# zhaoruiyang98/eftpipe

Measured on AMD Instinct MI355X. Metric: theory P_l(k) evaluations/sec (single tracer, Nk=512, l=0,2,4), higher is better.
Workload: dtype f64

## Files before the change

### eftpipe_amd/csrc/eftb_kernels.hpp

```cpp
#pragma once
#include <hip/hip_runtime.h>
#include <stdint.h>
#include <stdlib.h>

namespace eftb {

constexpr int NS = 80;
constexpr int NPOW = 257;
constexpr int NHALF = 128;
constexpr int NCH = 129;

constexpr int NROW = 24;

typedef double v4d __attribute__((ext_vector_type(4)));
typedef double v2d __attribute__((ext_vector_type(2)));

__device__ __forceinline__ void xcd_decode(int ntile, int& tile, int& group) {
    const int flat = blockIdx.x, ng = gridDim.x / ntile;
    if ((ng & 7) == 0) {
        const int slot = flat >> 3;
        tile = slot % ntile;
        group = (flat & 7) + 8 * (slot / ntile);
    } else {
        tile = flat % ntile;
        group = flat / ntile;
    }
}

template <bool LO>
__device__ __forceinline__ void prep_rows_body(int Nkin, int ntail, int nxtail, int KP1, int KP2, int KP3, int Bmax,
                                                        const double* __restrict__ Pin, const double* __restrict__ lnkin,
                                                        const double* __restrict__ lnxtail, const double* __restrict__ lnxxtail,
                                                        const double* __restrict__ wq2, double* __restrict__ A1, double* __restrict__ A2,
                                                        double* __restrict__ A2T, double* __restrict__ A3, int* __restrict__ status,
                                                        int ntail_lo, int nxtail_lo) {
    extern __shared__ double sm[];
    double* pin = sm;
    const int w = blockIdx.x, tid = threadIdx.x;
    bool bad = false;
    for (int j = tid; j < Nkin; j += blockDim.x) {
        const double v = Pin[(size_t)w * Nkin + j];
        pin[j] = v;
        bad = bad || !(fabs(v) <= 1.79769313486231570815e308) || (j >= Nkin - 2 && !(v > 0.0));
        if (LO) bad = bad || (j < 2 && !(v > 0.0));
    }
    if (bad && status) atomicMax(status, w + 1);
    __syncthreads();
    const double dln = lnkin[Nkin - 1] - lnkin[Nkin - 2];
    const double dlo = LO ? lnkin[1] - lnkin[0] : 0.0;
    if (A1) {
        const double slope = (log(pin[Nkin - 1]) - log(pin[Nkin - 2])) / dln;
        const double amp = pin[Nkin - 1] * exp(-slope * lnkin[Nkin - 1]);
        double slo = 0.0, alo = 0.0;
        if (LO && ntail_lo) {
            slo = (log(pin[1]) - log(pin[0])) / dlo;
            alo = pin[0] * exp(-slo * lnkin[0]);
        }
        const int nhi = ntail - (LO ? ntail_lo : 0);
        for (int j = tid; j < KP1; j += blockDim.x) A1[(size_t)w * KP1 + j] = j < Nkin ? pin[j] : 0.0;
        for (int j = tid; j < KP2; j += blockDim.x) {
            double v = j < Nkin ? pin[j] : (j < Nkin + ntail ? amp * exp(slope * lnxtail[j - Nkin]) : 0.0);
            if (LO && j >= Nkin + nhi && j < Nkin + ntail) v = alo * exp(slo * lnxtail[j - Nkin]);
            A2[(size_t)w * KP2 + j] = v;
            A2T[(size_t)j * Bmax + w] = v;
        }
    }
    if (A3) {
        const double q1 = pin[Nkin - 1] * wq2[1], q0 = pin[Nkin - 2] * wq2[0];
        const double slope = (log(q1) - log(q0)) / dln;
        const double amp = q1 * exp(-slope * lnkin[Nkin - 1]);
        double slo = 0.0, alo = 0.0;
        if (LO && nxtail_lo) {
            const double p0 = pin[0] * wq2[2], p1 = pin[1] * wq2[3];
            slo = (log(p1) - log(p0)) / dlo;
            alo = p0 * exp(-slo * lnkin[0]);
        }
        const int nhi = nxtail - (LO ? nxtail_lo : 0);
        for (int j = tid; j < KP3; j += blockDim.x) {
            double v = j < Nkin ? pin[j] : (j < Nkin + nxtail ? amp * exp(slope * lnxxtail[j - Nkin]) : 0.0);
            if (LO && j >= Nkin + nhi && j < Nkin + nxtail) v = alo * exp(slo * lnxxtail[j - Nkin]);
            A3[(size_t)w * KP3 + j] = v;
        }
    }
}

#define PREP_ROWS_PARAMS int Nkin, int ntail, int nxtail, int KP1, int KP2, int KP3, int Bmax, const double* __restrict__ Pin, \
    const double* __restrict__ lnkin, const double* __restrict__ lnxtail, const double* __restrict__ lnxxtail, const double* __restrict__ wq2, \
    double* __restrict__ A1, double* __restrict__ A2, double* __restrict__ A2T, double* __restrict__ A3, int* __restrict__ status
#define PREP_ROWS_ARGS Nkin, ntail, nxtail, KP1, KP2, KP3, Bmax, Pin, lnkin, lnxtail, lnxxtail, wq2, A1, A2, A2T, A3, status

__global__ __launch_bounds__(256) void prep_rows_kernel(PREP_ROWS_PARAMS) {
    prep_rows_body<false>(PREP_ROWS_ARGS, 0, 0);
}

__global__ __launch_bounds__(256) void prep_rows_lo_kernel(PREP_ROWS_PARAMS, int ntail_lo, int nxtail_lo) {
    prep_rows_body<true>(PREP_ROWS_ARGS, ntail_lo, nxtail_lo);
}

__device__ __forceinline__ void qf_body(int w, int nq, const double* __restrict__ fgrow, const double* __restrict__ Qpoly, double* __restrict__ Q) {
    const int tid = threadIdx.x;
    const double f = fgrow[w];
    for (int idx = tid; idx < 2 * nq; idx += blockDim.x) {
        const int a = idx / nq, rest = idx % nq;
        const double* c = Qpoly + ((size_t)(1 - a) * nq + rest) * 15;
        double cv[15];
#pragma unroll
        for (int p = 0; p < 15; ++p) cv[p] = c[p];
        const double f2 = f * f;
        double ev = cv[14], od = cv[13];
#pragma unroll
        for (int p = 12; p >= 0; p -= 2) {
            ev = fma(ev, f2, cv[p]);
            if (p >= 1) od = fma(od, f2, cv[p - 1]);
        }
        Q[(size_t)w * 2 * nq + idx] = fma(od, f, ev);
    }
}

__global__ __launch_bounds__(256) void prep_rows_qf_kernel(int B, PREP_ROWS_PARAMS, int nq, const double* __restrict__ fgrow,
                                                           const double* __restrict__ Qpoly, double* __restrict__ Q) {
    if ((int)blockIdx.x >= B) {
        qf_body(blockIdx.x - B, nq, fgrow, Qpoly, Q);
        return;
    }
    prep_rows_body<false>(PREP_ROWS_ARGS, 0, 0);
}

__global__ __launch_bounds__(256) void prep_rows_qf_lo_kernel(int B, PREP_ROWS_PARAMS, int nq, const double* __restrict__ fgrow,
                                                              const double* __restrict__ Qpoly, double* __restrict__ Q, int ntail_lo, int nxtail_lo) {
    if ((int)blockIdx.x >= B) {
        qf_body(blockIdx.x - B, nq, fgrow, Qpoly, Q);
        return;
    }
    prep_rows_body<true>(PREP_ROWS_ARGS, ntail_lo, nxtail_lo);
}
#undef PREP_ROWS_PARAMS
#undef PREP_ROWS_ARGS

constexpr int AD_T = NHALF + 2;
constexpr int AD_CH = 1;
constexpr int KSYN = 528;
constexpr int KLIN = 288;
constexpr int SYN_KPAD = 48;
constexpr int SYN_KC = 24;
static_assert(SYN_KPAD % SYN_KC == 0 && (32 * SYN_KC) % 256 == 0, "chunk must divide the padding and fill the staging threads");
constexpr int BAS22 = 8, BASC = 32;

__device__ __forceinline__ double readlane_f64(double v, int lane) {
    return __hiloint2double(__builtin_amdgcn_readlane(__double2hiint(v), lane), __builtin_amdgcn_readlane(__double2loint(v), lane));
}

template <int NC, int NW>
__global__ __launch_bounds__(64 * NW) void antidiag_kernel(int B, int Bmax, const double* __restrict__ coefT,
                                                           const double2* __restrict__ AD, double2* __restrict__ S) {
    constexpr int PB = 3, WPP = 2 * NC;
    static_assert(PB * WPP <= 64, "one wave-load must hold a block's weights");
    __shared__ double red[NW - 1][2 * NC][64];
    const int grp = blockIdx.y, jp = (grp & 1) ? NPOW - 1 - (int)blockIdx.x : (int)blockIdx.x;
    const int lane = threadIdx.x & 63, wave = threadIdx.x >> 6, w = grp * 64 + lane;
    const int wl = w < B ? w : B - 1;
    const int cnt = ((2 * NHALF + jp) >> 1) - jp + 1;
    const int per = (cnt + NW - 1) / NW, t0 = wave * per, t1 = min(cnt, t0 + per);
    const double* cr = coefT + wl;
    const double* ci = coefT + (size_t)NCH * Bmax + wl;
    double ar[NC], ai[NC];
#pragma unroll
    for (int q = 0; q < NC; ++q) ar[q] = ai[q] = 0.0;
    if (t0 < t1) {
        const double* adw = reinterpret_cast<const double*>(AD + ((size_t)jp * AD_T + t0) * NC);
        const int nw = (t1 - t0) * WPP;
        auto wload = [&](int blk) { return adw[min(blk * PB * WPP + lane, nw - 1)]; };
        double xr[PB], xi[PB], yr[PB], yi[PB];
        auto coef = [&](int t, int p) {
            const int n = jp + t, qn = n <= NHALF ? n : 2 * NHALF - n;
            xr[p] = cr[(size_t)qn * Bmax];
            xi[p] = ci[(size_t)qn * Bmax];
            yr[p] = cr[(size_t)t * Bmax];
            yi[p] = ci[(size_t)t * Bmax];
        };
        double wc = wload(0);
#pragma unroll
        for (int p = 0; p < PB; ++p) coef(min(t0 + p, t1 - 1), p);
        const int nblk = (t1 - t0 + PB - 1) / PB;
        for (int blk = 0; blk < nblk; ++blk) {
            const double wn = wload(blk + 1);
#pragma unroll
            for (int p = 0; p < PB; ++p) {
                const int t = t0 + blk * PB + p;
                const double on = t < t1 ? 1.0 : 0.0;
                const double xim = jp + t <= NHALF ? xi[p] : -xi[p], yim = -yi[p];
                const double pr = (xr[p] * yr[p] - xim * yim) * on, pi = (xr[p] * yim + xim * yr[p]) * on;
                __builtin_amdgcn_sched_barrier(0);
                coef(min(t + PB, t1 - 1), p);
                __builtin_amdgcn_sched_barrier(0);
#pragma unroll
                for (int q = 0; q < NC; ++q) {
                    const double mx = readlane_f64(wc, p * WPP + 2 * q), my = readlane_f64(wc, p * WPP + 2 * q + 1);
                    ar[q] = fma(mx, pr, fma(-my, pi, ar[q]));
                    ai[q] = fma(mx, pi, fma(my, pr, ai[q]));
                }
                __builtin_amdgcn_sched_barrier(0);
            }
            wc = wn;
        }
    }
    if (wave > 0) {
#pragma unroll
        for (int q = 0; q < NC; ++q) {
            red[wave - 1][2 * q][lane] = ar[q];
            red[wave - 1][2 * q + 1][lane] = ai[q];
        }
    }
    __syncthreads();
    if (wave == 0 && w < B) {
#pragma unroll
        for (int q = 0; q < NC; ++q) {
#pragma unroll
            for (int v = 0; v < NW - 1; ++v) {
                ar[q] += red[v][2 * q][lane];
                ai[q] += red[v][2 * q + 1][lane];
            }
            S[((size_t)w * NC + q) * NPOW + jp] = make_double2(ar[q], ai[q]);
        }
    }
}

template <int NC, int NW>
__global__ __launch_bounds__(64 * NW) void antidiag_nh_kernel(int B, int Bmax, const double* __restrict__ coefT,
                                                              const double2* __restrict__ AD, double2* __restrict__ S, int nh) {
    constexpr int PB = 3, WPP = 2 * NC;
    static_assert(PB * WPP <= 64, "one wave-load must hold a block's weights");
    __shared__ double red[NW - 1][2 * NC][64];
    const int npow = 2 * nh + 1, nch = nh + 1, adt = nh + 2;
    const int grp = blockIdx.y, jp = (grp & 1) ? npow - 1 - (int)blockIdx.x : (int)blockIdx.x;
    const int lane = threadIdx.x & 63, wave = threadIdx.x >> 6, w = grp * 64 + lane;
    const int wl = w < B ? w : B - 1;
    const int cnt = ((2 * nh + jp) >> 1) - jp + 1;
    const int per = (cnt + NW - 1) / NW, t0 = wave * per, t1 = min(cnt, t0 + per);
    const double* cr = coefT + wl;
    const double* ci = coefT + (size_t)nch * Bmax + wl;
    double ar[NC], ai[NC];
#pragma unroll
    for (int q = 0; q < NC; ++q) ar[q] = ai[q] = 0.0;
    if (t0 < t1) {
        const double* adw = reinterpret_cast<const double*>(AD + ((size_t)jp * adt + t0) * NC);
        const int nw = (t1 - t0) * WPP;
        auto wload = [&](int blk) { return adw[min(blk * PB * WPP + lane, nw - 1)]; };
        double xr[PB], xi[PB], yr[PB], yi[PB];
        auto coef = [&](int t, int p) {
            const int n = jp + t, qn = n <= nh ? n : 2 * nh - n;
            xr[p] = cr[(size_t)qn * Bmax];
            xi[p] = ci[(size_t)qn * Bmax];
            yr[p] = cr[(size_t)t * Bmax];
            yi[p] = ci[(size_t)t * Bmax];
        };
        double wc = wload(0);
#pragma unroll
        for (int p = 0; p < PB; ++p) coef(min(t0 + p, t1 - 1), p);
        const int nblk = (t1 - t0 + PB - 1) / PB;
        for (int blk = 0; blk < nblk; ++blk) {
            const double wn = wload(blk + 1);
#pragma unroll
            for (int p = 0; p < PB; ++p) {
                const int t = t0 + blk * PB + p;
                const double on = t < t1 ? 1.0 : 0.0;
                const double xim = jp + t <= nh ? xi[p] : -xi[p], yim = -yi[p];
                const double pr = (xr[p] * yr[p] - xim * yim) * on, pi = (xr[p] * yim + xim * yr[p]) * on;
                __builtin_amdgcn_sched_barrier(0);
                coef(min(t + PB, t1 - 1), p);
                __builtin_amdgcn_sched_barrier(0);
#pragma unroll
                for (int q = 0; q < NC; ++q) {
                    const double mx = readlane_f64(wc, p * WPP + 2 * q), my = readlane_f64(wc, p * WPP + 2 * q + 1);
                    ar[q] = fma(mx, pr, fma(-my, pi, ar[q]));
                    ai[q] = fma(mx, pi, fma(my, pr, ai[q]));
                }
                __builtin_amdgcn_sched_barrier(0);
            }
            wc = wn;
        }
    }
    if (wave > 0) {
#pragma unroll
        for (int q = 0; q < NC; ++q) {
            red[wave - 1][2 * q][lane] = ar[q];
            red[wave - 1][2 * q + 1][lane] = ai[q];
        }
    }
    __syncthreads();
    if (wave == 0 && w < B) {
#pragma unroll
        for (int q = 0; q < NC; ++q) {
#pragma unroll
            for (int v = 0; v < NW - 1; ++v) {
                ar[q] += red[v][2 * q][lane];
                ai[q] += red[v][2 * q + 1][lane];
            }
            S[((size_t)w * NC + q) * npow + jp] = make_double2(ar[q], ai[q]);
        }
    }
}

template <int NC>
__global__ __launch_bounds__(64) void build_rows_kernel(int sets, int Bmax, int Nl, int nlc, int nb, const double* __restrict__ coef,
                                                         const double2* __restrict__ S, const double2* __restrict__ mlj,
                                                         const double2* __restrict__ linvec, double* __restrict__ A22,
                                                         double* __restrict__ A13, double* __restrict__ ACF, double* __restrict__ ALC) {
    const int w = blockIdx.x, cf = blockIdx.y, jp = blockIdx.z * 64 + threadIdx.x;
    if (((sets >> cf) & 1) && jp < NPOW) {
        double zr[NC], zi[NC];
#pragma unroll
        for (int q = 0; q < NC; ++q) {
            zr[q] = zi[q] = 0.0;
#pragma unroll
            for (int ch = 0; ch < AD_CH; ++ch) {
                const double2 v = S[(((size_t)ch * Bmax + w) * NC + q) * NPOW + jp];
                zr[q] += v.x;
                zi[q] += v.y;
            }
        }
        const int o0 = jp == 0 ? 0 : 2 * jp - 1;
        if (cf == 0) {
#pragma unroll
            for (int q = 0; q < NC; ++q)
                if (q < nb) {
                    double* o = A22 + ((size_t)w * BAS22 + q) * KSYN;
                    o[o0] = zr[q];
                    if (jp) o[o0 + 1] = zi[q];
                }
        } else {
            for (int l = 0; l < Nl; ++l) {
                const double2 m = mlj[l * NPOW + jp];
#pragma unroll
                for (int q = 0; q < NC; ++q) {
                    double* o = ACF + ((size_t)w * BASC + l * NC + q) * KSYN;
                    o[o0] = m.x * zr[q] - m.y * zi[q];
                    if (jp) o[o0 + 1] = m.x * zi[q] + m.y * zr[q];
                }
            }
        }
    }
    if ((sets >> (2 + cf)) & 1) {
        const int nrows = cf == 0 ? 10 : nlc * Nl, v0 = cf == 0 ? 0 : 10;
        double* out = cf == 0 ? A13 + (size_t)w * 10 * KLIN : ALC + (size_t)w * nlc * Nl * KLIN;
        const double* c = coef + (size_t)w * 2 * NCH;
        for (int e = jp; e < nrows * NCH; e += 320) {
            const int row = e / NCH, mp = e % NCH, n = NHALF - mp;
            const double2 v = linvec[(size_t)(v0 + row) * NCH + n];
            const double cr = c[n], ci = n == NHALF ? 0.0 : c[NCH + n];
            double* o = out + (size_t)row * KLIN;
            if (mp == 0) o[0] = cr * v.x - ci * v.y;
            else {
                o[2 * mp - 1] = cr * v.x - ci * v.y;
                o[2 * mp] = cr * v.y + ci * v.x;
            }
        }
    }
}

__host__ __device__ constexpr int ksyn_of(int nh) { return (4 * nh + SYN_KPAD) / SYN_KPAD * SYN_KPAD; }
__host__ __device__ constexpr int klin_of(int nh) { return (2 * nh + SYN_KPAD) / SYN_KPAD * SYN_KPAD; }
static_assert(ksyn_of(NHALF) == KSYN && klin_of(NHALF) == KLIN, "row lengths of the default NFFT");

template <int NC>
__global__ __launch_bounds__(64) void build_rows_nh_kernel(int sets, int Bmax, int Nl, int nlc, int nb, const double* __restrict__ coef,
                                                            const double2* __restrict__ S, const double2* __restrict__ mlj,
                                                            const double2* __restrict__ linvec, double* __restrict__ A22,
                                                            double* __restrict__ A13, double* __restrict__ ACF, double* __restrict__ ALC, int nh) {
    const int npow = 2 * nh + 1, nch = nh + 1, ksyn = ksyn_of(nh), klin = klin_of(nh), zstride = 64 * (int)gridDim.z;
    const int w = blockIdx.x, cf = blockIdx.y, jp = blockIdx.z * 64 + threadIdx.x;
    if (((sets >> cf) & 1) && jp < npow) {
        double zr[NC], zi[NC];
#pragma unroll
        for (int q = 0; q < NC; ++q) {
            zr[q] = zi[q] = 0.0;
#pragma unroll
            for (int ch = 0; ch < AD_CH; ++ch) {
                const double2 v = S[(((size_t)ch * Bmax + w) * NC + q) * npow + jp];
                zr[q] += v.x;
                zi[q] += v.y;
            }
        }
        const int o0 = jp == 0 ? 0 : 2 * jp - 1;
        if (cf == 0) {
#pragma unroll
            for (int q = 0; q < NC; ++q)
                if (q < nb) {
                    double* o = A22 + ((size_t)w * BAS22 + q) * ksyn;
                    o[o0] = zr[q];
                    if (jp) o[o0 + 1] = zi[q];
                }
        } else {
            for (int l = 0; l < Nl; ++l) {
                const double2 m = mlj[l * npow + jp];
#pragma unroll
                for (int q = 0; q < NC; ++q) {
                    double* o = ACF + ((size_t)w * BASC + l * NC + q) * ksyn;
                    o[o0] = m.x * zr[q] - m.y * zi[q];
                    if (jp) o[o0 + 1] = m.x * zi[q] + m.y * zr[q];
                }
            }
        }
    }
    if ((sets >> (2 + cf)) & 1) {
        const int nrows = cf == 0 ? 10 : nlc * Nl, v0 = cf == 0 ? 0 : 10;
        double* out = cf == 0 ? A13 + (size_t)w * 10 * klin : ALC + (size_t)w * nlc * Nl * klin;
        const double* c = coef + (size_t)w * 2 * nch;
        for (int e = jp; e < nrows * nch; e += zstride) {
            const int row = e / nch, mp = e % nch, n = nh - mp;
            const double2 v = linvec[(size_t)(v0 + row) * nch + n];
            const double cr = c[n], ci = n == nh ? 0.0 : c[nch + n];
            double* o = out + (size_t)row * klin;
            if (mp == 0) o[0] = cr * v.x - ci * v.y;
            else {
                o[2 * mp - 1] = cr * v.x - ci * v.y;
                o[2 * mp] = cr * v.y + ci * v.x;
            }
        }
    }
}

__device__ inline double ipow(double f, int p) {
    double r = 1.0;
    for (int i = 0; i < p; ++i) r *= f;
    return r;
}

template <int NC>
__global__ __launch_bounds__(64) void build_rows_plk_kernel(int Bmax, int nb, const double* __restrict__ coef, const double2* __restrict__ S,
                                                             const double2* __restrict__ mlj, const double2* __restrict__ linvec,
                                                             const double* __restrict__ bias, const double* __restrict__ fgrow,
                                                             const double* __restrict__ l11, const double* __restrict__ lct,
                                                             const double* __restrict__ l22, const double* __restrict__ l13,
                                                             const int* __restrict__ grp, const double* __restrict__ exp22,
                                                             const double* __restrict__ expc, double* __restrict__ A22, double* __restrict__ A13,
                                                             double* __restrict__ ACF, double* __restrict__ ALC) {
    constexpr int NL = 3;
    __shared__ double s_cf[NL * 38];
    __shared__ double s_w[NL * NC];
    __shared__ double s_b[2 * NL];
    const int w = blockIdx.x, cf = blockIdx.y, jp = blockIdx.z * 64 + threadIdx.x;
    const double* bw = bias + (size_t)w * NROW;
    const double f = fgrow[w];
    for (int e = threadIdx.x; e < NL * 38; e += 64) {
        const int l = e / 38, bq = e % 38;
        s_cf[e] = bw[9 + grp[2 * bq]] * ipow(f, grp[2 * bq + 1]) * (bq < 28 ? l22[l * 28 + bq] : l13[l * 10 + (bq - 28)]);
    }
    if (threadIdx.x < 2 * NL) {
        const int a = threadIdx.x / NL, lp = threadIdx.x % NL;
        double v = 0.0;
        if (a == 0)
            for (int r = 0; r < 3; ++r) v = fma(bw[r], l11[lp * 3 + r], v);
        else
            for (int r = 0; r < 6; ++r) v = fma(bw[3 + r], lct[lp * 6 + r], v);
        s_b[threadIdx.x] = v;
    }
    __syncthreads();
    if (threadIdx.x < NL * NC) {
        const int l = threadIdx.x / NC, q = threadIdx.x % NC;
        double v0 = 0.0, v1 = 0.0;
        if (cf == 0) {
            if (q < nb)
                for (int b = 0; b < 28; b += 2) {
                    v0 = fma(s_cf[l * 38 + b], exp22[b * BAS22 + q], v0);
                    v1 = fma(s_cf[l * 38 + b + 1], exp22[(b + 1) * BAS22 + q], v1);
                }
        } else {
            for (int b = 0; b < 28; b += 2) {
                v0 = fma(s_cf[l * 38 + b], expc[(size_t)(l * 28 + b) * BASC + l * NC + q], v0);
                v1 = fma(s_cf[l * 38 + b + 1], expc[(size_t)(l * 28 + b + 1) * BASC + l * NC + q], v1);
            }
            for (int b = 0; b < 10; b += 2) {
                v0 = fma(s_cf[l * 38 + 28 + b], expc[(size_t)(NL * 28 + l * 10 + b) * BASC + l * NC + q], v0);
                v1 = fma(s_cf[l * 38 + 29 + b], expc[(size_t)(NL * 28 + l * 10 + b + 1) * BASC + l * NC + q], v1);
            }
        }
        s_w[threadIdx.x] = v0 + v1;
    }
    __syncthreads();
    if (jp < NPOW) {
        double zr[NC], zi[NC];
#pragma unroll
        for (int q = 0; q < NC; ++q) {
            zr[q] = zi[q] = 0.0;
#pragma unroll
            for (int ch = 0; ch < AD_CH; ++ch) {
                const double2 v = S[(((size_t)ch * Bmax + w) * NC + q) * NPOW + jp];
                zr[q] += v.x;
                zi[q] += v.y;
            }
        }
        const int o0 = jp == 0 ? 0 : 2 * jp - 1;
#pragma unroll
        for (int l = 0; l < NL; ++l) {
            double cr = 0.0, ci = 0.0;
#pragma unroll
            for (int q = 0; q < NC; ++q) {
                cr = fma(s_w[l * NC + q], zr[q], cr);
                ci = fma(s_w[l * NC + q], zi[q], ci);
            }
            if (cf == 0) {
                double* o = A22 + ((size_t)w * BAS22 + l) * KSYN;
                o[o0] = cr;
                if (jp) o[o0 + 1] = ci;
            } else {
                const double2 m = mlj[l * NPOW + jp];
                double* o = ACF + ((size_t)w * BASC + l) * KSYN;
                o[o0] = m.x * cr - m.y * ci;
                if (jp) o[o0 + 1] = m.x * ci + m.y * cr;
            }
        }
    }
    {
        const int nrows = cf == 0 ? NL : 2 * NL;
        double* out = cf == 0 ? A13 + (size_t)w * 10 * KLIN : ALC + (size_t)w * 2 * NL * KLIN;
        const double* c = coef + (size_t)w * 2 * NCH;
        for (int e = jp; e < nrows * NCH; e += 320) {
            const int row = e / NCH, mp = e % NCH, n = NHALF - mp;
            double vx, vy;
            if (cf == 0) {
                vx = vy = 0.0;
#pragma unroll
                for (int b = 0; b < 10; ++b) {
                    const double2 v = linvec[(size_t)b * NCH + n];
                    vx = fma(s_cf[row * 38 + 28 + b], v.x, vx);
                    vy = fma(s_cf[row * 38 + 28 + b], v.y, vy);
                }
            } else {
                const double2 v = linvec[(size_t)(10 + row) * NCH + n];
                vx = s_b[row] * v.x;
                vy = s_b[row] * v.y;
            }
            const double cr = c[n], ci = n == NHALF ? 0.0 : c[NCH + n];
            double* o = out + (size_t)row * KLIN;
            if (mp == 0) o[0] = cr * vx - ci * vy;
            else {
                o[2 * mp - 1] = cr * vx - ci * vy;
                o[2 * mp] = cr * vy + ci * vx;
            }
        }
    }
}

template <int NC>
__global__ __launch_bounds__(64) void build_rows_plk_nh_kernel(int Bmax, int nb, const double* __restrict__ coef, const double2* __restrict__ S,
                                                    const double2* __restrict__ mlj, const double2* __restrict__ linvec,
                                                    const double* __restrict__ bias, const double* __restrict__ fgrow,
                                                    const double* __restrict__ l11, const double* __restrict__ lct,
                                                    const double* __restrict__ l22, const double* __restrict__ l13,
                                                    const int* __restrict__ grp, const double* __restrict__ exp22,
                                                    const double* __restrict__ expc, double* __restrict__ A22, double* __restrict__ A13,
                                                    double* __restrict__ ACF, double* __restrict__ ALC, int nh) {
    constexpr int NL = 3;
    const int npow = 2 * nh + 1, nch = nh + 1, ksyn = ksyn_of(nh), klin = klin_of(nh), zstride = 64 * (int)gridDim.z;
    __shared__ double s_cf[NL * 38];
    __shared__ double s_w[NL * NC];
    __shared__ double s_b[2 * NL];
    const int w = blockIdx.x, cf = blockIdx.y, jp = blockIdx.z * 64 + threadIdx.x;
    const double* bw = bias + (size_t)w * NROW;
    const double f = fgrow[w];
    for (int e = threadIdx.x; e < NL * 38; e += 64) {
        const int l = e / 38, bq = e % 38;
        s_cf[e] = bw[9 + grp[2 * bq]] * ipow(f, grp[2 * bq + 1]) * (bq < 28 ? l22[l * 28 + bq] : l13[l * 10 + (bq - 28)]);
    }
    if (threadIdx.x < 2 * NL) {
        const int a = threadIdx.x / NL, lp = threadIdx.x % NL;
        double v = 0.0;
        if (a == 0)
            for (int r = 0; r < 3; ++r) v = fma(bw[r], l11[lp * 3 + r], v);
        else
            for (int r = 0; r < 6; ++r) v = fma(bw[3 + r], lct[lp * 6 + r], v);
        s_b[threadIdx.x] = v;
    }
    __syncthreads();
    if (threadIdx.x < NL * NC) {
        const int l = threadIdx.x / NC, q = threadIdx.x % NC;
        double v0 = 0.0, v1 = 0.0;
        if (cf == 0) {
            if (q < nb)
                for (int b = 0; b < 28; b += 2) {
                    v0 = fma(s_cf[l * 38 + b], exp22[b * BAS22 + q], v0);
                    v1 = fma(s_cf[l * 38 + b + 1], exp22[(b + 1) * BAS22 + q], v1);
                }
        } else {
            for (int b = 0; b < 28; b += 2) {
                v0 = fma(s_cf[l * 38 + b], expc[(size_t)(l * 28 + b) * BASC + l * NC + q], v0);
                v1 = fma(s_cf[l * 38 + b + 1], expc[(size_t)(l * 28 + b + 1) * BASC + l * NC + q], v1);
            }
            for (int b = 0; b < 10; b += 2) {
                v0 = fma(s_cf[l * 38 + 28 + b], expc[(size_t)(NL * 28 + l * 10 + b) * BASC + l * NC + q], v0);
                v1 = fma(s_cf[l * 38 + 29 + b], expc[(size_t)(NL * 28 + l * 10 + b + 1) * BASC + l * NC + q], v1);
            }
        }
        s_w[threadIdx.x] = v0 + v1;
    }
    __syncthreads();
    if (jp < npow) {
        double zr[NC], zi[NC];
#pragma unroll
        for (int q = 0; q < NC; ++q) {
            zr[q] = zi[q] = 0.0;
#pragma unroll
            for (int ch = 0; ch < AD_CH; ++ch) {
// ... 3766 lines not shown
```

Before: 1.854 million.

## Load antidiagonal weights as wave-uniform scalars and double-buffer coefficient prefetch

The antidiagonal kernels now share one body templated on a compile-time half size. Each wave reads its per-step weights through a uniform address (wave index made scalar with readfirstlane), so the compiler can use scalar loads instead of a lane-indexed vector load followed by readlane broadcasts. The weight and coefficient loads are double-buffered two steps ahead. The tail masking multiply is dropped in favour of an explicit remainder step, and the sign flip becomes a bit xor. The aim is fewer VALU/readlane instructions per MAC and better load latency hiding, at the cost of more scalar registers and reliance on inline-asm scheduling hints.

```diff
diff --git a/eftpipe_amd/csrc/eftb_kernels.hpp b/eftpipe_amd/csrc/eftb_kernels.hpp
--- a/eftpipe_amd/csrc/eftb_kernels.hpp
+++ b/eftpipe_amd/csrc/eftb_kernels.hpp
@@ -150,155 +150,117 @@
     return __hiloint2double(__builtin_amdgcn_readlane(__double2hiint(v), lane), __builtin_amdgcn_readlane(__double2loint(v), lane));
 }
 
+template <int NC, int NW, int NH>
+__device__ __forceinline__ void antidiag_body(int B, int Bmax, const double* __restrict__ coefT, const double2* __restrict__ AD,
+                                              double2* __restrict__ S, int nh_rt, double (&red)[NW - 1][2 * NC][64]) {
+    constexpr int WPP = 2 * NC;
+    const int nh = NH ? NH : nh_rt, npow = 2 * nh + 1, nch = nh + 1, adt = nh + 2;
+    const int grp = blockIdx.y, jp = (grp & 1) ? npow - 1 - (int)blockIdx.x : (int)blockIdx.x;
+    const int lane = threadIdx.x & 63, wave = __builtin_amdgcn_readfirstlane(threadIdx.x >> 6), w = grp * 64 + lane;
+    const int wl = w < B ? w : B - 1;
+    const int cnt = ((2 * nh + jp) >> 1) - jp + 1;
+    const int per = (cnt + NW - 1) / NW, t0 = wave * per, t1 = min(cnt, t0 + per);
+    double ar[NC], ai[NC];
+#pragma unroll
+    for (int q = 0; q < NC; ++q) ar[q] = ai[q] = 0.0;
+    if (t0 < t1) {
+        const double* adw = reinterpret_cast<const double*>(AD + (size_t)jp * adt * NC);
+        const char* cr = reinterpret_cast<const char*>(coefT);
+        const char* ci = reinterpret_cast<const char*>(coefT + (size_t)nch * Bmax);
+        const unsigned rowb = (unsigned)Bmax * 8u;
+        unsigned lo = (unsigned)wl * 8u;
+        double wa[WPP], wb[WPP], xr[2], xi[2], yr[2], yi[2];
+        auto weights = [&](double(&wv)[WPP], int t) {
+            const double* p = adw + (size_t)t * WPP;
+#pragma unroll
+            for (int j = 0; j < WPP; ++j) wv[j] = p[j];
+        };
+        auto row = [&](const char* base, int r) { return *reinterpret_cast<const double*>(base + (size_t)(unsigned)r * rowb + lo); };
+        auto coef = [&](int t, int p) {
+            const int n = jp + t, qn = n <= nh ? n : 2 * nh - n;
+            asm volatile("" : "+v"(lo));
+            xr[p] = row(cr, qn);
+            xi[p] = row(ci, qn);
+            yr[p] = row(cr, t);
+            yi[p] = row(ci, t);
+        };
+        double pr, pi;
+        auto products = [&](int t, int p) {
+            const unsigned sm = jp + t <= nh ? 0u : 0x80000000u;
+            const double xim = __hiloint2double(__double2hiint(xi[p]) ^ (int)sm, __double2loint(xi[p]));
+            pr = fma(xim, yi[p], xr[p] * yr[p]);
+            pi = fma(xim, yr[p], -(xr[p] * yi[p]));
+        };
+        auto macs = [&](const double(&wc)[WPP]) {
+#pragma unroll
+            for (int q = 0; q < NC; ++q) {
+                const double mx = wc[2 * q], my = wc[2 * q + 1];
+                ar[q] = fma(mx, pr, fma(-my, pi, ar[q]));
+                ai[q] = fma(mx, pi, fma(my, pr, ai[q]));
+            }
+        };
+#define AD_WAIT(x)                                                                     \
+    asm volatile("" ::"s"(x));  \
+    __builtin_amdgcn_sched_barrier(0)
+        auto step = [&](const double(&wc)[WPP], double(&wn)[WPP], int t, int p) {
+            products(t, p);
+            __builtin_amdgcn_sched_barrier(0);
+            coef(min(t + 2, t1 - 1), p);
+            __builtin_amdgcn_sched_barrier(0);
+            AD_WAIT(wc[0]);
+            weights(wn, min(t + 1, t1 - 1));
+            __builtin_amdgcn_sched_barrier(0);
+            macs(wc);
+            __builtin_amdgcn_sched_barrier(0);
+        };
+        weights(wa, t0);
+        coef(t0, 0);
+        coef(min(t0 + 1, t1 - 1), 1);
+        int t = t0;
+        for (; t + 1 < t1; t += 2) {
+            step(wa, wb, t, 0);
+            step(wb, wa, t + 1, 1);
+        }
+        if (t < t1) {
+            products(t, 0);
+            AD_WAIT(wa[0]);
+            macs(wa);
+        }
+#undef AD_WAIT
+    }
+    if (wave > 0) {
+#pragma unroll
+        for (int q = 0; q < NC; ++q) {
+            red[wave - 1][2 * q][lane] = ar[q];
+            red[wave - 1][2 * q + 1][lane] = ai[q];
+        }
+    }
+    __syncthreads();
+    if (wave == 0 && w < B) {
+#pragma unroll
+        for (int q = 0; q < NC; ++q) {
+#pragma unroll
+            for (int v = 0; v < NW - 1; ++v) {
+                ar[q] += red[v][2 * q][lane];
+                ai[q] += red[v][2 * q + 1][lane];
+            }
+            S[((size_t)w * NC + q) * npow + jp] = make_double2(ar[q], ai[q]);
+        }
+    }
+}
+
 template <int NC, int NW>
 __global__ __launch_bounds__(64 * NW) void antidiag_kernel(int B, int Bmax, const double* __restrict__ coefT,
                                                            const double2* __restrict__ AD, double2* __restrict__ S) {
-    constexpr int PB = 3, WPP = 2 * NC;
-    static_assert(PB * WPP <= 64, "one wave-load must hold a block's weights");
     __shared__ double red[NW - 1][2 * NC][64];
-    const int grp = blockIdx.y, jp = (grp & 1) ? NPOW - 1 - (int)blockIdx.x : (int)blockIdx.x;
-    const int lane = threadIdx.x & 63, wave = threadIdx.x >> 6, w = grp * 64 + lane;
-    const int wl = w < B ? w : B - 1;
-    const int cnt = ((2 * NHALF + jp) >> 1) - jp + 1;
-    const int per = (cnt + NW - 1) / NW, t0 = wave * per, t1 = min(cnt, t0 + per);
-    const double* cr = coefT + wl;
-    const double* ci = coefT + (size_t)NCH * Bmax + wl;
-    double ar[NC], ai[NC];
-#pragma unroll
-    for (int q = 0; q < NC; ++q) ar[q] = ai[q] = 0.0;
-    if (t0 < t1) {
-        const double* adw = reinterpret_cast<const double*>(AD + ((size_t)jp * AD_T + t0) * NC);
-        const int nw = (t1 - t0) * WPP;
-        auto wload = [&](int blk) { return adw[min(blk * PB * WPP + lane, nw - 1)]; };
-        double xr[PB], xi[PB], yr[PB], yi[PB];
-        auto coef = [&](int t, int p) {
-            const int n = jp + t, qn = n <= NHALF ? n : 2 * NHALF - n;
-            xr[p] = cr[(size_t)qn * Bmax];
-            xi[p] = ci[(size_t)qn * Bmax];
-            yr[p] = cr[(size_t)t * Bmax];
-            yi[p] = ci[(size_t)t * Bmax];
-        };
-        double wc = wload(0);
-#pragma unroll
-        for (int p = 0; p < PB; ++p) coef(min(t0 + p, t1 - 1), p);
-        const int nblk = (t1 - t0 + PB - 1) / PB;
-        for (int blk = 0; blk < nblk; ++blk) {
-            const double wn = wload(blk + 1);
-#pragma unroll
-            for (int p = 0; p < PB; ++p) {
-                const int t = t0 + blk * PB + p;
-                const double on = t < t1 ? 1.0 : 0.0;
-                const double xim = jp + t <= NHALF ? xi[p] : -xi[p], yim = -yi[p];
-                const double pr = (xr[p] * yr[p] - xim * yim) * on, pi = (xr[p] * yim + xim * yr[p]) * on;
-                __builtin_amdgcn_sched_barrier(0);
-                coef(min(t + PB, t1 - 1), p);
-                __builtin_amdgcn_sched_barrier(0);
-#pragma unroll
-                for (int q = 0; q < NC; ++q) {
-                    const double mx = readlane_f64(wc, p * WPP + 2 * q), my = readlane_f64(wc, p * WPP + 2 * q + 1);
-                    ar[q] = fma(mx, pr, fma(-my, pi, ar[q]));
-                    ai[q] = fma(mx, pi, fma(my, pr, ai[q]));
-                }
-                __builtin_amdgcn_sched_barrier(0);
-            }
-            wc = wn;
-        }
-    }
-    if (wave > 0) {
-#pragma unroll
-        for (int q = 0; q < NC; ++q) {
-            red[wave - 1][2 * q][lane] = ar[q];
-            red[wave - 1][2 * q + 1][lane] = ai[q];
-        }
-    }
-    __syncthreads();
-    if (wave == 0 && w < B) {
-#pragma unroll
-        for (int q = 0; q < NC; ++q) {
-#pragma unroll
-            for (int v = 0; v < NW - 1; ++v) {
-                ar[q] += red[v][2 * q][lane];
-                ai[q] += red[v][2 * q + 1][lane];
-            }
-            S[((size_t)w * NC + q) * NPOW + jp] = make_double2(ar[q], ai[q]);
-        }
-    }
+    antidiag_body<NC, NW, NHALF>(B, Bmax, coefT, AD, S, NHALF, red);
 }
 
 template <int NC, int NW>
 __global__ __launch_bounds__(64 * NW) void antidiag_nh_kernel(int B, int Bmax, const double* __restrict__ coefT,
                                                               const double2* __restrict__ AD, double2* __restrict__ S, int nh) {
-    constexpr int PB = 3, WPP = 2 * NC;
-    static_assert(PB * WPP <= 64, "one wave-load must hold a block's weights");
     __shared__ double red[NW - 1][2 * NC][64];
-    const int npow = 2 * nh + 1, nch = nh + 1, adt = nh + 2;
-    const int grp = blockIdx.y, jp = (grp & 1) ? npow - 1 - (int)blockIdx.x : (int)blockIdx.x;
-    const int lane = threadIdx.x & 63, wave = threadIdx.x >> 6, w = grp * 64 + lane;
-    const int wl = w < B ? w : B - 1;
-    const int cnt = ((2 * nh + jp) >> 1) - jp + 1;
-    const int per = (cnt + NW - 1) / NW, t0 = wave * per, t1 = min(cnt, t0 + per);
-    const double* cr = coefT + wl;
-    const double* ci = coefT + (size_t)nch * Bmax + wl;
-    double ar[NC], ai[NC];
-#pragma unroll
-    for (int q = 0; q < NC; ++q) ar[q] = ai[q] = 0.0;
-    if (t0 < t1) {
-        const double* adw = reinterpret_cast<const double*>(AD + ((size_t)jp * adt + t0) * NC);
-        const int nw = (t1 - t0) * WPP;
-        auto wload = [&](int blk) { return adw[min(blk * PB * WPP + lane, nw - 1)]; };
-        double xr[PB], xi[PB], yr[PB], yi[PB];
-        auto coef = [&](int t, int p) {
-            const int n = jp + t, qn = n <= nh ? n : 2 * nh - n;
-            xr[p] = cr[(size_t)qn * Bmax];
-            xi[p] = ci[(size_t)qn * Bmax];
-            yr[p] = cr[(size_t)t * Bmax];
-            yi[p] = ci[(size_t)t * Bmax];
-        };
-        double wc = wload(0);
-#pragma unroll
-        for (int p = 0; p < PB; ++p) coef(min(t0 + p, t1 - 1), p);
-        const int nblk = (t1 - t0 + PB - 1) / PB;
-        for (int blk = 0; blk < nblk; ++blk) {
-            const double wn = wload(blk + 1);
-#pragma unroll
-            for (int p = 0; p < PB; ++p) {
-                const int t = t0 + blk * PB + p;
-                const double on = t < t1 ? 1.0 : 0.0;
-                const double xim = jp + t <= nh ? xi[p] : -xi[p], yim = -yi[p];
-                const double pr = (xr[p] * yr[p] - xim * yim) * on, pi = (xr[p] * yim + xim * yr[p]) * on;
-                __builtin_amdgcn_sched_barrier(0);
-                coef(min(t + PB, t1 - 1), p);
-                __builtin_amdgcn_sched_barrier(0);
-#pragma unroll
-                for (int q = 0; q < NC; ++q) {
-                    const double mx = readlane_f64(wc, p * WPP + 2 * q), my = readlane_f64(wc, p * WPP + 2 * q + 1);
-                    ar[q] = fma(mx, pr, fma(-my, pi, ar[q]));
-                    ai[q] = fma(mx, pi, fma(my, pr, ai[q]));
-                }
-                __builtin_amdgcn_sched_barrier(0);
-            }
-            wc = wn;
-        }
-    }
-    if (wave > 0) {
-#pragma unroll
-        for (int q = 0; q < NC; ++q) {
-            red[wave - 1][2 * q][lane] = ar[q];
-            red[wave - 1][2 * q + 1][lane] = ai[q];
-        }
-    }
-    __syncthreads();
-    if (wave == 0 && w < B) {
-#pragma unroll
-        for (int q = 0; q < NC; ++q) {
-#pragma unroll
-            for (int v = 0; v < NW - 1; ++v) {
-                ar[q] += red[v][2 * q][lane];
-                ai[q] += red[v][2 * q + 1][lane];
-            }
-            S[((size_t)w * NC + q) * npow + jp] = make_double2(ar[q], ai[q]);
-        }
-    }
+    antidiag_body<NC, NW, 0>(B, Bmax, coefT, AD, S, nh, red);
 }
 
 template <int NC>
```

New measurement: 1.845 million. Within noise of the previous version (-0.5%).
